# Lornatang/Real_ESRGAN-PyTorch

Hardware: AMD Instinct MI355X
Metric: x4 SR train images/sec (256->1024) (higher is better)
Workload: dtype f16; 1 GPU; RealESRNet x4 L1 train step, RRDBNet 23 blocks, LR 256^2 -> HR 1024^2, batch 16/GPU, degradation=hip, Adam+EMA, GradScaler; global_batch=16, parallelism=dp1

## Files before the change

real_esrgan-pytorch_amd/csrc/build.py:

```python
import os
import subprocess
import sys
from concurrent.futures import ThreadPoolExecutor

HERE = os.path.dirname(os.path.abspath(__file__))
ROOT = os.path.dirname(os.path.dirname(HERE))
SOURCES = ["api.hip", "conv3x3.hip", "conv3x3_ws.hip", "conv3x3_ws_mt1.hip", "conv3x3_ws_mt2.hip", "conv3x3_ws_x2_mt1.hip", "conv3x3_ws_x2_mt2.hip", "conv3x3_ws_sp.hip", "conv3x3_ws_chain.hip", "conv3x3_ws_chain_x2.hip", "wgrad.hip", "pack.hip", "layout.hip", "generator.hip", "degrade.hip", "degrade_int.hip", "disc.hip", "disc_native.hip", "loss.hip", "sustained.hip"]
LIB = os.path.join(HERE, "libresr_hip.so")
HIPCC = os.environ.get("HIPCC", "/opt/rocm/bin/hipcc")
FLAGS = ["--offload-arch=gfx950", "-O3", "-std=c++17", "-fPIC", "-I", os.path.join(ROOT, "include"), "-I", HERE,
         "-Wno-unused-result"]


def _stale(target, deps):
    if not os.path.exists(target):
        return True
    t = os.path.getmtime(target)
    return any(os.path.getmtime(d) > t for d in deps)


def build(force=False, verbose=False):
    hdrs = [os.path.join(HERE, "common.h"), os.path.join(HERE, "conv3x3.h"), os.path.join(HERE, "conv3x3_ws.h"), os.path.join(HERE, "conv3x3_ws_chain.h"), os.path.join(HERE, "wgrad.h"), os.path.join(ROOT, "include", "resr.h"), os.path.join(ROOT, "include", "resr_debug.h"), os.path.abspath(__file__)]
    extra = [s for s in os.listdir(HERE) if s.endswith(".hip") and s not in SOURCES]
    srcs = SOURCES + sorted(extra)
    objs, jobs = [], []
    for s in srcs:
        src = os.path.join(HERE, s)
        obj = os.path.join(HERE, s.replace(".hip", ".o"))
        objs.append(obj)
        if force or _stale(obj, [src] + hdrs):
            cmd = [HIPCC] + FLAGS + ["-c", src, "-o", obj]
            if verbose:
                cmd.insert(1, "-Rpass-analysis=kernel-resource-usage")
            jobs.append(cmd)

    def run(cmd):
        r = subprocess.run(cmd, capture_output=True, text=True)
        return cmd, r

    with ThreadPoolExecutor(max_workers=6) as ex:
        for cmd, r in ex.map(run, jobs):
            if verbose or r.returncode:
                sys.stderr.write(" ".join(cmd) + "\n" + r.stdout + r.stderr)
            if r.returncode:
                raise RuntimeError("hipcc failed: " + " ".join(cmd))
    if force or jobs or _stale(LIB, objs):
        cmd = [HIPCC, "--offload-arch=gfx950", "-shared", "-fPIC", "-o", LIB] + objs
        r = subprocess.run(cmd, capture_output=True, text=True)
        if r.returncode:
            sys.stderr.write(r.stdout + r.stderr)
            raise RuntimeError("link failed")
    return LIB


if __name__ == "__main__":
    print(build(force="--force" in sys.argv, verbose="--verbose" in sys.argv))
```

real_esrgan-pytorch_amd/csrc/generator.hip:

```cpp
#include <stdlib.h>
#include <vector>

#include "common.h"
#include "wgrad.h"

namespace resr {

int conv3x3_dispatch(const ResrConvDesc*, const void*, const void*, const void*, const float*, const void*,
                     const void*, const void*, void*, void*, hipStream_t);
size_t wgrad_batch_partial_bytes(const WgradConv*, int, int, int);
int conv3x3_block_dispatch(int njobs, const ResrConvDesc* d, const void* in0, const void* in1, const void* const* w,
                           const float* const* bias, const void* const* mask, void* const* out, void* const* aux,
                           const ResrConvDesc* d5, const void* w5, const float* bias5, const void* res0_5, const void* res1_5,
                           void* out5, void* chain_state, size_t chain_state_bytes, hipStream_t stream);
size_t conv3x3_chain_state_bytes(int, int, int);
int wgrad_batch(const WgradConv*, int, int, int, int, int, int, int, float*, hipStream_t);
int wgrad_batch_jobs(const WgradConv*, int, int);
int wgrad_batch_quads(const WgradConv*, int, int);
int wgrad_tile_rows(int dtype);
int wgrad_x2_products();
int nchw_to_nhwc_dispatch(const float*, void*, int, int, int, int, int, int, int, const uint8_t*, hipStream_t, long);
int nhwc_to_nchw_dispatch(const void*, float*, int, int, int, int, int, int, int, hipStream_t, long);
int absmax_dispatch(const float*, long, unsigned*, int, hipStream_t);
int nchw_to_nhwc_scaled_dispatch(const float*, void*, int, int, int, int, int, int, int, const uint8_t*, hipStream_t, long, const unsigned*);
int nchw_to_nhwc_q_dispatch(const float*, void*, int, int, int, int, int, int, int, const uint8_t*, hipStream_t, long, const unsigned*, long);
int nhwc_to_nchw_scaled_dispatch(const void*, float*, int, int, int, int, int, int, int, hipStream_t, long, const unsigned*);
int sumpool2x2_dispatch(const void*, void*, const void*, int, int, int, int, int, float, hipStream_t, long, long);
int add_inplace_dispatch(void*, const void*, long, int, hipStream_t, long, long);

namespace {

struct ConvSpec {
    int cout, cin, cin_pad, cout_pad;
    size_t w_off, b_off;
    size_t pk_fwd, pk_bwd;
};

struct Plan {
    ResrGeneratorDesc d;
    int r;
    int h, w;
    int ci_real, ci_pad;
    int nrdb;
    std::vector<ConvSpec> convs;
    size_t n_params;
    size_t pk_fwd_elems, pk_total_elems;
    int i_conv1, i_trunk0, i_conv2, i_up1, i_up2, i_conv3, i_conv4;
    std::vector<size_t> pk_bwd_trunk;
    size_t pk_bwd_conv4, pk_bwd_conv3, pk_bwd_up2, pk_bwd_up1, pk_bwd_conv2, pk_bwd_conv1;
};

int round32(int v) { return (v + 31) / 32 * 32; }

bool plan_mx_bwd(const ResrGeneratorDesc& d) {
    return d.dtype == RESR_F16X2 && d.training && (d.x2_plan & RESR_X2_PLAN_MX_BWD) && !(d.x2_plan & RESR_X2_PLAN_GROWTH_GRAD_STORE_F16);
}
bool plan_mx_wgrad(const ResrGeneratorDesc& d) {
    return plan_mx_bwd(d) && (d.x2_plan & RESR_X2_PLAN_MX_WGRAD) && !(d.x2_plan & RESR_X2_PLAN_F16_BACKWARD);
}
bool plan_mx_tail(const ResrGeneratorDesc& d) { return plan_mx_wgrad(d) && (d.x2_plan & RESR_X2_PLAN_MX_TAIL); }
constexpr int kMxTrainNeeds = RESR_X2_PLAN_GROWTH_F16_INFER | RESR_X2_PLAN_GROWTH_W16_INFER | RESR_X2_PLAN_MX_INFER | RESR_X2_PLAN_F16_BACKWARD;
bool plan_mx_train(const ResrGeneratorDesc& d) {
    return d.dtype == RESR_F16X2 && d.training && (d.x2_plan & RESR_X2_PLAN_MX_TRAIN_FORWARD) && (d.x2_plan & kMxTrainNeeds) == kMxTrainNeeds;
}
bool plan_mx_train_ok(const ResrGeneratorDesc& d) {
    return d.dtype != RESR_F16X2 || !(d.x2_plan & RESR_X2_PLAN_MX_TRAIN_FORWARD) || (d.x2_plan & kMxTrainNeeds) == kMxTrainNeeds;
}
bool plan_mx(const ResrGeneratorDesc& d) {
    const int need = RESR_X2_PLAN_GROWTH_F16_INFER | RESR_X2_PLAN_GROWTH_W16_INFER | RESR_X2_PLAN_MX_INFER;
    return (d.dtype == RESR_F16X2 && !d.training && (d.x2_plan & need) == need) || plan_mx_train(d);
}

bool build_plan(const ResrGeneratorDesc* d, Plan& p) {
    if (!d) return false;
    if (d->upscale != 4 && d->upscale != 2 && d->upscale != 1) return false;
    if (d->n <= 0 || d->h <= 0 || d->w <= 0 || d->n_blocks <= 0 || d->in_channels <= 0 || d->out_channels <= 0) return false;
    p.d = *d;
    p.r = d->upscale == 4 ? 1 : (d->upscale == 2 ? 2 : 4);
    if ((d->h % p.r) || (d->w % p.r)) return false;
    p.h = d->h / p.r;
    p.w = d->w / p.r;
    p.ci_real = d->in_channels * p.r * p.r;
    p.ci_pad = round32(p.ci_real);
    if (p.ci_pad > 64 || d->out_channels > 32) return false;
    p.nrdb = d->n_blocks * 3;
    size_t off = 0;
    auto add = [&](int cout, int cin) {
        ConvSpec c;
        c.cout = cout; c.cin = cin; c.cin_pad = round32(cin); c.cout_pad = round32(cout);
        c.w_off = off; off += (size_t)cout * cin * 9;
        c.b_off = off; off += cout;
        c.pk_fwd = c.pk_bwd = 0;
        p.convs.push_back(c);
        return (int)p.convs.size() - 1;
    };
    p.i_conv1 = add(64, p.ci_real);
    p.i_trunk0 = (int)p.convs.size();
    for (int r = 0; r < p.nrdb; ++r)
        for (int k = 1; k <= 5; ++k) add(k < 5 ? 32 : 64, 64 + 32 * (k - 1));
    p.i_conv2 = add(64, 64);
    p.i_up1 = add(64, 64);
    p.i_up2 = add(64, 64);
    p.i_conv3 = add(64, 64);
    p.i_conv4 = add(d->out_channels, 64);
    p.n_params = off;
    size_t pk = 0;
    for (auto& c : p.convs) {
        c.pk_fwd = pk;
        pk += (size_t)(c.cin_pad / 32) * 9 * (c.cout_pad / 32) * 1024;
    }
    p.pk_fwd_elems = pk;
    auto bwd_simple = [&](int idx) {
        const ConvSpec& c = p.convs[idx];
        const size_t o = pk;
        pk += (size_t)(c.cout_pad / 32) * 9 * (c.cin_pad / 32) * 1024;
        return o;
    };
    p.pk_bwd_conv4 = bwd_simple(p.i_conv4);
    p.pk_bwd_conv3 = bwd_simple(p.i_conv3);
    p.pk_bwd_up2 = bwd_simple(p.i_up2);
    p.pk_bwd_up1 = bwd_simple(p.i_up1);
    p.pk_bwd_conv2 = bwd_simple(p.i_conv2);
    p.pk_bwd_conv1 = bwd_simple(p.i_conv1);
    p.pk_bwd_trunk.resize((size_t)p.nrdb * 5);
    for (int r = 0; r < p.nrdb; ++r)
        for (int ps = 0; ps < 5; ++ps) {
            p.pk_bwd_trunk[(size_t)r * 5 + ps] = pk;
            pk += (size_t)(2 + ps) * 9 * (ps < 4 ? 1 : 2) * 1024;
        }
    p.pk_total_elems = pk;
    return true;
}

struct Bufs {
    char* chain;
    size_t chain_bytes;
    char* x_in;
    std::vector<char*> ws;
    char *bits_u2, *bits_c3;
    std::vector<char*> bits;
    char* out1;
    int out1_stride;
    char *trunk_out, *feat, *u1, *u2, *c3;
    uint8_t* ymask;
    char *g4, *gA, *gB, *gM1, *gF, *gT[4], *gS[3], *gxin;
    float* partial;
    size_t partial_bytes;
    unsigned* gscale;
    size_t total;
};

int splits_for(const Plan& p, int npairs, int h, int w, int nquads = 0) {
    if (p.d.wgrad_splits > 0) return p.d.wgrad_splits;
    const int th = wgrad_tile_rows(p.d.dtype);
    const long tiles = (long)((w + 31) / 32) * ((h + th - 1) / th) * p.d.n;
    if (p.d.dtype == RESR_F16X2 && nquads > 0 && tiles >= 64 && !getenv("RESR_X2_WGRAD_OLD_SPLITS")) {
        long best_s = 8;
        double best = 1e30;
        for (long s = 8; s <= 256 && s <= tiles / 2; s += 8) {
            const long rounds = (nquads * (s / 8) + 31) / 32;
            const double cost = rounds * ((double)tiles / s * 2.9 + 8.0) + (double)npairs * s * 0.0185;
            if (cost < best) { best = cost; best_s = s; }
        }
        return (int)best_s;
    }
    long s;
    if (p.d.dtype != RESR_F32) {
        s = 512 / ((npairs + 3) / 4);
        if (s >= 16) s &= ~7L;
        if (s > 256) s = 256;
    } else {
        s = 768 / npairs;
        if (s > 128) s = 128;
    }
    if (s > tiles / 2) s = tiles / 2;
    if (s < 1) s = 1;
    return (int)s;
}

void carve(const Plan& p, char* base, Bufs& b) {
    const size_t es = elem_size(p.d.dtype) * (act_tensors(p.d.dtype) + (plan_mx(p.d) ? 1 : 0));
// ... 294 lines not shown
                outs4[k - 1] = cur + (size_t)(2 + (k - 1)) * plane * es; signs4[k - 1] = signs;
            }
            const ConvSpec& c = p.convs[p.i_trunk0 + r * 5 + 4];
            const bool last = r == p.nrdb - 1;
            char* dst = last ? b.trunk_out : b.ws[(r + 1) % nws];
            ResrConvDesc cd = conv_desc(p, N, h, w, 192, 192, 32, 0, 64, 64, 32, 0);
            cd.in0_chunk_stride = plane;
            cd.out_chunk_stride = plane;
            cd.in0_lo_offset = lo_ws; cd.out_lo_offset = last ? lo_t : lo_ws;
            if (growth_single) { cd.x2_pair_chunks = 2; if (growth_w16) cd.flags |= RESR_CONV_SINGLE_W16; }
            MXP(cd, c, 2 * lo_ws, last ? 2 * lo_t : 2 * lo_ws);
            if (mxw && !last) cd.out_q_offset = 2 * lo_ws;
            cd.s0 = 0.2f; cd.t0 = 1.f; cd.res0_stride = 32; cd.res0_chunk_stride = plane; cd.res0_lo_offset = lo_ws;
            const char* res1 = nullptr;
            if (r % 3 == 2) {
                res1 = b.ws[(r - 2) % nws];
                cd.s1 = 0.2f; cd.t1 = 1.f; cd.res1_stride = 32; cd.res1_chunk_stride = plane; cd.res1_lo_offset = lo_ws;
            }
            RUN(conv3x3_block_dispatch(4, cds, cur, nullptr, ws4, bs4, nullptr, outs4, signs4, &cd, W(c), Bias(c), cur, res1, dst, b.chain, b.chain_bytes, st));
        }
    }
    {
        const ConvSpec& c = p.convs[p.i_conv2];
        ResrConvDesc cd = conv_desc(p, N, h, w, 64, 64, 32, 0, 64, 64, 64, 0);
        cd.in0_chunk_stride = plane;
        cd.res0_stride = b.out1_stride;
        cd.res0_chunk_stride = b.out1 == b.ws[0] ? plane : 0;
        cd.out_stride = 32; cd.out_chunk_stride = plane;
        cd.in0_lo_offset = lo_t; cd.res0_lo_offset = lo_out1; cd.out_lo_offset = lo_t;
        MXP(cd, c, 2 * lo_t, 2 * lo_t);
        RUN(conv3x3_dispatch(&cd, b.trunk_out, nullptr, W(c), Bias(c), b.out1, nullptr, nullptr, b.feat, nullptr, st));
    }
    {
        const ConvSpec& c = p.convs[p.i_up1];
        ResrConvDesc cd = conv_desc(p, N, 2 * h, 2 * w, 64, 64, 32, 0, 64, 64, 32, RESR_CONV_LRELU | RESR_CONV_UPSAMPLE_IN);
        cd.in0_chunk_stride = plane; cd.out_chunk_stride = 4 * plane;
        cd.in0_lo_offset = lo_t; cd.out_lo_offset = LO(2, 4L * plane);
        MXP(cd, c, 2 * lo_t, 2 * LO(2, 4L * plane));
        if (mxt) cd.out_q_offset = 2 * LO(2, 4L * plane);
        RUN(conv3x3_dispatch(&cd, b.feat, nullptr, W(c), Bias(c), nullptr, nullptr, nullptr, b.u1, nullptr, st));
    }
    {
        const ConvSpec& c = p.convs[p.i_up2];
        ResrConvDesc cd = conv_desc(p, N, 4 * h, 4 * w, 64, 64, 32, 0, 64, 64, 32, RESR_CONV_LRELU | RESR_CONV_UPSAMPLE_IN);
        cd.in0_chunk_stride = 4 * plane; cd.out_chunk_stride = 16 * plane;
        cd.in0_lo_offset = LO(2, 4L * plane); cd.out_lo_offset = LO(2, 16L * plane);
        if (d->training) cd.flags |= RESR_CONV_WRITE_SIGNBITS;
        MXP(cd, c, 2 * LO(2, 4L * plane), 2 * LO(2, 16L * plane));
        if (mxt) cd.out_q_offset = 2 * LO(2, 16L * plane);
        RUN(conv3x3_dispatch(&cd, b.u1, nullptr, W(c), Bias(c), nullptr, nullptr, nullptr, b.u2, b.bits_u2, st));
    }
    {
        const ConvSpec& c = p.convs[p.i_conv3];
        ResrConvDesc cd = conv_desc(p, N, 4 * h, 4 * w, 64, 64, 32, 0, 64, 64, 32, RESR_CONV_LRELU);
        cd.in0_chunk_stride = 16 * plane; cd.out_chunk_stride = 16 * plane;
        cd.in0_lo_offset = LO(2, 16L * plane); cd.out_lo_offset = LO(2, 16L * plane);
        if (d->training) cd.flags |= RESR_CONV_WRITE_SIGNBITS;
        MXP(cd, c, 2 * LO(2, 16L * plane), 0);
        if (mxt) cd.out_q_offset = 2 * LO(2, 16L * plane);
        RUN(conv3x3_dispatch(&cd, b.u2, nullptr, W(c), Bias(c), nullptr, nullptr, nullptr, b.c3, b.bits_c3, st));
    }
    {
        const ConvSpec& c = p.convs[p.i_conv4];
        ResrConvDesc cd = conv_desc(p, N, 4 * h, 4 * w, 64, 64, 32, 0, c.cout, c.cout_pad, 0,
                                    RESR_CONV_CLAMP01 | RESR_CONV_OUT_NCHW_F32);
        cd.in0_chunk_stride = 16 * plane;
        cd.in0_lo_offset = LO(2, 16L * plane);
        RUN(conv3x3_dispatch(&cd, b.c3, nullptr, W(c), Bias(c), nullptr, nullptr, nullptr, y, b.ymask, st));
    }
    return RESR_OK;
}

int generator_backward(const ResrGeneratorDesc* d, const float* gy, const float* params, const void* packed,
                       void* workspace, size_t workspace_bytes, float* grad, float* gx, hipStream_t st,
                       void* const* events, int n_events) {
    (void)params;
    Plan p;
    if (!build_plan(d, p)) return fail(RESR_ERR_ARG, "generator_backward: bad descriptor");
    if (!plan_mx_train_ok(*d)) return fail(RESR_ERR_ARG, "generator_backward: x2_plan MX_TRAIN_FORWARD (2048) needs bits 1 + 32 + 64 + 256");
    if (n_events != 0 && (!events || n_events != d->n_blocks + 2))
        return fail(RESR_ERR_ARG, "generator_backward: grad_ready_events needs n_blocks + 2 = %d events, got %d", d->n_blocks + 2, n_events);
    auto ready = [&](int i) -> int {
        if (n_events == 0) return RESR_OK;
        if (!events[i]) return fail(RESR_ERR_ARG, "generator_backward: null event %d", i);
        if (hipEventRecord((hipEvent_t)events[i], st) != hipSuccess) return fail(RESR_ERR_LAUNCH, "generator_backward: hipEventRecord");
        return RESR_OK;
    };
    if (!d->training) return fail(RESR_ERR_ARG, "generator_backward: forward was not run with training=1");
    if (!gy || !packed || !workspace || !grad) return fail(RESR_ERR_ARG, "generator_backward: null argument");
    Bufs b;
    carve(p, (char*)workspace, b);
    if (b.total > workspace_bytes) return fail(RESR_ERR_WORKSPACE, "generator_backward: workspace %zu < %zu", workspace_bytes, b.total);
    const bool f16bwd = d->dtype == RESR_F16X2 && (d->x2_plan & RESR_X2_PLAN_F16_BACKWARD);
    const int dt = f16bwd ? (int)RESR_F16 : d->dtype;
    Plan pb = p;
    pb.d.dtype = dt;
    const size_t es = elem_size(dt);
    const bool x2 = dt == RESR_F16X2;
    const size_t wes = es * (x2 ? 3 : 1);
    const int wm = x2 ? wgrad_x2_products() : 1;
    const char* no_prescale = getenv("RESR_X2_NO_GRAD_PRESCALE");
    const char* pre_t = getenv("RESR_X2_GRAD_PRESCALE_LOG2");
    const int pre_log2 = pre_t ? atoi(pre_t) : 6;
    const unsigned* gsc = (dt != RESR_F32 && !no_prescale) ? b.gscale : nullptr;
    const bool mxb = plan_mx_bwd(*d) && !f16bwd;
    const bool mxw = plan_mx_wgrad(*d) && mxb;
    const bool mxt = plan_mx_tail(*d) && mxw;
    const bool gg_single = x2 && (d->x2_plan & RESR_X2_PLAN_GROWTH_GRAD_F16);
    const bool gg_store_single = gg_single && (d->x2_plan & RESR_X2_PLAN_GROWTH_GRAD_STORE_F16);
    const int wx_pairs = (x2 && (d->x2_plan & RESR_X2_PLAN_GROWTH_ACT_F16_WGRAD)) ? 2 : 0;
    const char* pk = (const char*)packed;
    const int N = d->n, h = p.h, w = p.w;
    const int H4 = 4 * h, W4 = 4 * w, H2 = 2 * h, W2 = 2 * w;
    if ((long)N * h * w * 32 * 16 > 0x7fffffffL) return fail(RESR_ERR_ARG, "generator: batch x resolution too large for 32-bit chunk strides");
    const int plane = N * h * w * 32;
    const int pl2 = 4 * plane, pl4 = 16 * plane;
    auto LO = [&](long planes, long pl) -> long { return x2 ? planes * pl : 0; };
    const long lo_ws = LO(6, plane), lo_t = LO(2, plane), lo_gs = LO(4, plane), lo_2 = LO(2, pl2), lo_4 = LO(2, pl4), lo_g4 = LO(1, pl4);
    const long lo_xin = x2 ? (long)N * h * w * p.ci_pad : 0;

    auto wconv = [&](const ConvSpec& c, const void* x0, int cin, int s0, const void* g, int gstride, float scale,
                     long x_lo, long g_lo) {
        WgradConv wc;
        wc.x0 = x0; wc.cin = cin; wc.in0_stride = s0; wc.cin_real = c.cin;
        wc.g = g; wc.cout = c.cout; wc.cout_pad = c.cout_pad; wc.g_stride = gstride;
        wc.x_chunk_stride = wc.g_chunk_stride = 0;
        wc.x_lo_off = x_lo; wc.g_lo_off = g_lo; wc.x_s2d_c = 0; wc.g_lo_bias_only = 0;
        wc.dw = grad + c.w_off; wc.db = grad + c.b_off; wc.scale = scale;
        wc.unscale = gsc;
        return wc;
    };
    auto wgrad_run = [&](const WgradConv* wc, int nconv, int hh, int ww, int flags) -> int {
        const int njobs = wgrad_batch_jobs(wc, nconv, dt);
        const int splits = splits_for(pb, njobs, hh, ww, x2 ? wgrad_batch_quads(wc, nconv, dt) : 0);
        if (wgrad_batch_partial_bytes(wc, nconv, splits, dt) > b.partial_bytes)
            return fail(RESR_ERR_WORKSPACE, "wgrad slab buffer too small");
        return wgrad_batch(wc, nconv, N, hh, ww, dt, flags, splits, b.partial, st);
    };
    auto wgrad = [&](const ConvSpec& c, int hh, int ww, const void* x0, int cin, int s0, const void* g, int gstride,
                     int flags, float scale, long x_chunk, long g_chunk, long x_lo, long g_lo, long x_q = 0, long g_q = 0) -> int {
        WgradConv wc = wconv(c, x0, cin, s0, g, gstride, scale, x_lo, g_lo);
        wc.x_chunk_stride = x_chunk; wc.g_chunk_stride = g_chunk;
        wc.x_q_off = x_q; wc.g_q_off = g_q;
        return wgrad_run(&wc, 1, hh, ww, flags);
    };
    auto dgrad = [&](int hh, int ww, int cin0, int s0, int cin, int s1, int cout, int cout_pad, int out_stride, int flags,
                     long lo0, long lo1, long lo_out) {
        ResrConvDesc cd = conv_desc(pb, N, hh, ww, cin, cin0, s0, s1, cout, cout_pad, out_stride, flags | RESR_CONV_NO_BIAS);
        cd.in0_lo_offset = lo0; cd.in1_lo_offset = lo1; cd.out_lo_offset = lo_out;
        return cd;
    };

    if (gsc) RUN(absmax_dispatch(gy, (long)N * d->out_channels * H4 * W4, b.gscale, pre_log2, st));
    RUN(nchw_to_nhwc_q_dispatch(gy, b.g4, N, d->out_channels, H4, W4, 1, 32, dt, b.ymask, st, lo_g4, gsc, mxt ? 2 * lo_g4 : 0L));
    const char* pk_mx = mxb ? pk + generator_mx_offset(d) : nullptr;
    auto MXT = [&](ResrConvDesc& cd, size_t pk_off, long in_q, long out_q) {
        if (!mxt) return;
        cd.flags |= RESR_CONV_MX_PAIRS;
        cd.in0_q_offset = in_q; cd.out_q_offset = out_q;
        cd.w_mx_offset = (int64_t)((pk_mx + pk_off * 2) - (pk + pk_off * wes));
    };
    {
        const ConvSpec& c = p.convs[p.i_conv4];
        RUN(wgrad(c, H4, W4, b.c3, 64, 32, b.g4, 32, 0, 1.f, pl4, 0, lo_4, lo_g4, mxt ? 2 * lo_4 : 0, mxt ? 2 * lo_g4 : 0));
        ResrConvDesc cd = dgrad(H4, W4, 32, 32, 32, 0, 64, 64, 32, RESR_CONV_MASK | RESR_CONV_MASK_BITS, lo_g4, 0, lo_4);
        cd.out_chunk_stride = pl4;
        MXT(cd, p.pk_bwd_conv4, 2 * lo_g4, 2 * lo_4);
        RUN(conv3x3_dispatch(&cd, b.g4, nullptr, pk + p.pk_bwd_conv4 * wes, nullptr, nullptr, nullptr, b.bits_c3, b.gA, nullptr, st));
    }
    {
        const ConvSpec& c = p.convs[p.i_conv3];
        RUN(wgrad(c, H4, W4, b.u2, 64, 32, b.gA, 32, 0, 1.f, pl4, pl4, lo_4, lo_4, mxt ? 2 * lo_4 : 0, mxt ? 2 * lo_4 : 0));
        ResrConvDesc cd = dgrad(H4, W4, 64, 32, 64, 0, 64, 64, 32, RESR_CONV_MASK | RESR_CONV_MASK_BITS, lo_4, 0, lo_4);
        cd.in0_chunk_stride = pl4; cd.out_chunk_stride = pl4;
        MXT(cd, p.pk_bwd_conv3, 2 * lo_4, 2 * lo_4);
        RUN(conv3x3_dispatch(&cd, b.gA, nullptr, pk + p.pk_bwd_conv3 * wes, nullptr, nullptr, nullptr, b.bits_u2, b.gB, nullptr, st));
    }
    if (debug_stop() == 1) return RESR_OK;
    {
        const ConvSpec& c = p.convs[p.i_up2];
        RUN(wgrad(c, H4, W4, b.u1, 64, 32, b.gB, 32, RESR_CONV_UPSAMPLE_IN, 1.f, pl2, pl4, lo_2, lo_4, mxt ? 2 * lo_2 : 0, mxt ? 2 * lo_4 : 0));
        ResrConvDesc cd = dgrad(H4, W4, 64, 32, 64, 0, 64, 64, 32, 0, lo_4, 0, lo_4);
        cd.in0_chunk_stride = pl4; cd.out_chunk_stride = pl4;
        MXT(cd, p.pk_bwd_up2, 2 * lo_4, 0);
        RUN(conv3x3_dispatch(&cd, b.gB, nullptr, pk + p.pk_bwd_up2 * wes, nullptr, nullptr, nullptr, nullptr, b.gA, nullptr, st));
        for (int q = 0; q < 2; ++q)
            RUN(sumpool2x2_dispatch(b.gA + (size_t)q * pl4 * es, b.gM1 + (size_t)q * pl2 * es, b.u1 + (size_t)q * pl2 * es,
                                    N, H2, W2, 32, dt, 0.2f, st, lo_4, lo_2));
    }
    if (debug_stop() == 2) return RESR_OK;
    {
        const ConvSpec& c = p.convs[p.i_up1];
        RUN(wgrad(c, H2, W2, b.feat, 64, 32, b.gM1, 32, RESR_CONV_UPSAMPLE_IN, 1.f, plane, pl2, lo_t, lo_2));
        ResrConvDesc cd = dgrad(H2, W2, 64, 32, 64, 0, 64, 64, 32, 0, lo_2, 0, lo_2);
        cd.in0_chunk_stride = pl2; cd.out_chunk_stride = pl2;
        RUN(conv3x3_dispatch(&cd, b.gM1, nullptr, pk + p.pk_bwd_up1 * wes, nullptr, nullptr, nullptr, nullptr, b.gA, nullptr, st));
        for (int q = 0; q < 2; ++q)
            RUN(sumpool2x2_dispatch(b.gA + (size_t)q * pl2 * es, b.gF + (size_t)q * plane * es, nullptr, N, h, w, 32, dt, 0.2f, st,
                                    lo_2, lo_t));
    }
    if (debug_stop() == 3) return RESR_OK;
    int cur = 0;
    {
        const ConvSpec& c = p.convs[p.i_conv2];
        RUN(wgrad(c, h, w, b.trunk_out, 64, 32, b.gF, 32, 0, 1.f, plane, plane, lo_t, lo_t));
        ResrConvDesc cd = dgrad(h, w, 64, 32, 64, 0, 64, 64, 32, 0, lo_t, 0, lo_t);
        cd.in0_chunk_stride = plane; cd.out_chunk_stride = plane;
        if (mxb) cd.out_q_offset = 2 * lo_t;
        RUN(conv3x3_dispatch(&cd, b.gF, nullptr, pk + p.pk_bwd_conv2 * wes, nullptr, nullptr, nullptr, nullptr, b.gT[0], nullptr, st));
    }
    auto MXB = [&](ResrConvDesc& cd, size_t pk_off, long out_q) {
        if (!mxb) return;
        cd.flags |= RESR_CONV_MX_PAIRS;
        cd.x2_pair_chunks = 0;
        cd.in0_q_offset = 2 * lo_t; cd.in1_q_offset = 2 * lo_gs; cd.out_q_offset = out_q;
        cd.w_mx_offset = (int64_t)((pk_mx + pk_off * 2) - (pk + pk_off * wes));
    };
    RUN(ready(0));
    int e_idx = 0;
    const bool batch_rrdb = 78 * wm <= kWgradMaxJobs && !getenv("RESR_WGRAD_PER_BLOCK");
    WgradConv wc[15];
    for (int r = p.nrdb - 1; r >= 0; --r) {
        const int pos = r % 3;
        if (pos == 2) e_idx = cur;
        const char* gin = b.gT[cur];
        const char* act = b.ws[r];
        char* gS = b.gS[pos];
        const float fold = pos == 2 ? 0.04f : 0.2f;
        WgradConv* wcb = wc + (batch_rrdb ? 5 * pos : 0);
        wcb[4] = wconv(p.convs[p.i_trunk0 + r * 5 + 4], act, 192, 32, gin, 32, fold, lo_ws, lo_t);
        wcb[4].x_chunk_stride = plane; wcb[4].g_chunk_stride = plane;
        wcb[4].x_pair_chunks = wx_pairs;
        wcb[4].x_single_g_hi = (wx_pairs && (d->x2_plan & RESR_X2_PLAN_GROWTH_ACT_G_HI_WGRAD)) ? 1 : 0;
        if (mxw) { wcb[4].x_q_off = 2 * lo_ws; wcb[4].g_q_off = 2 * lo_t; }
        ResrConvDesc cds[4];
        const void* ws4[4];
        const void* masks4[4];
        void* outs4[4];
        for (int ps = 0; ps < 4; ++ps) {
            const int k = 4 - ps;
            const int cin = 64 + 32 * ps;
            ResrConvDesc cd = dgrad(h, w, 64, 32, cin, 32, 32, 32, 32, RESR_CONV_MASK | RESR_CONV_MASK_BITS, lo_t, lo_gs, lo_gs);
            cd.in0_chunk_stride = plane; cd.in1_chunk_stride = plane;
            if (gg_single) cd.x2_pair_chunks = 2;
            if (gg_store_single) cd.flags |= RESR_CONV_OUT_SINGLE;
            MXB(cd, p.pk_bwd_trunk[(size_t)r * 5 + ps], 2 * lo_gs);
            char* out = gS + (size_t)ps * plane * es;
            const char* mask = b.bits[r] + (size_t)(k - 1) * N * h * w * sizeof(uint32_t);
            cds[ps] = cd; ws4[ps] = pk + p.pk_bwd_trunk[(size_t)r * 5 + ps] * wes; masks4[ps] = mask; outs4[ps] = out;
            const ConvSpec& c = p.convs[p.i_trunk0 + r * 5 + k - 1];
            wcb[k - 1] = wconv(c, act, c.cin, 32, out, 32, 1.f, lo_ws, gg_store_single ? 0 : lo_gs);
            wcb[k - 1].x_chunk_stride = plane;
            wcb[k - 1].g_lo_bias_only = (gg_single && !gg_store_single) ? 1 : 0;
            wcb[k - 1].x_pair_chunks = wx_pairs;
            if (mxw) { wcb[k - 1].x_q_off = 2 * lo_ws; wcb[k - 1].g_q_off = 2 * lo_gs; }
        }
        {
            int nxt = (cur + 1) & 3;
            if (nxt == e_idx && pos != 2) nxt = (nxt + 1) & 3;
            ResrConvDesc cd = dgrad(h, w, 64, 32, 192, 32, 64, 64, 32, 0, lo_t, lo_gs, lo_t);
            cd.in0_chunk_stride = plane; cd.in1_chunk_stride = plane; cd.out_chunk_stride = plane;
            if (gg_single) cd.x2_pair_chunks = 2;
            const char* res0 = gin;
            const char* res1 = nullptr;
            cd.res0_stride = 32; cd.res0_chunk_stride = plane; cd.s0 = 1.f; cd.res0_lo_offset = lo_t;
            cd.t0 = pos == 2 ? 0.2f : 1.f;
            if (pos == 0) { res1 = b.gT[e_idx]; cd.res1_stride = 32; cd.res1_chunk_stride = plane; cd.s1 = 1.f; cd.t1 = 1.f; cd.res1_lo_offset = lo_t; }
            MXB(cd, p.pk_bwd_trunk[(size_t)r * 5 + 4], 2 * lo_t);
            RUN(conv3x3_block_dispatch(4, cds, gin, gS, ws4, nullptr, masks4, outs4, nullptr, &cd,
                                       pk + p.pk_bwd_trunk[(size_t)r * 5 + 4] * wes, nullptr, res0, res1, b.gT[nxt], b.chain, b.chain_bytes, st));
            cur = nxt;
        }
        if (!batch_rrdb) RUN(wgrad_run(wc, 5, h, w, 0));
        else if (pos == 0) RUN(wgrad_run(wc, 15, h, w, 0));
        if (pos == 0) RUN(ready(1 + (d->n_blocks - 1 - r / 3)));
    }
    if (debug_stop() == 4) return RESR_OK;
    RUN(add_inplace_dispatch(b.gT[cur], b.gF, (long)N * h * w * 64, dt, st, lo_t, lo_t));
    {
        const ConvSpec& c = p.convs[p.i_conv1];
        RUN(wgrad(c, h, w, b.x_in, p.ci_pad, p.ci_pad, b.gT[cur], 32, 0, 1.f, 0, plane, lo_xin, lo_t));
        RUN(ready(d->n_blocks + 1));
        if (gx) {
            ResrConvDesc cd = dgrad(h, w, 64, 32, 64, 0, p.ci_pad, p.ci_pad, p.ci_pad, 0, lo_t, 0, lo_xin);
            cd.in0_chunk_stride = plane;
            RUN(conv3x3_dispatch(&cd, b.gT[cur], nullptr, pk + p.pk_bwd_conv1 * wes, nullptr, nullptr, nullptr, nullptr, b.gxin, nullptr, st));
            RUN(nhwc_to_nchw_scaled_dispatch(b.gxin, gx, N, d->in_channels, d->h, d->w, p.r, p.ci_pad, dt, st, lo_xin, gsc));
        }
    }
    return RESR_OK;
}

}
```

Before: 131.0 images/sec.

## Add compact 4-channel tail backward kernels for final 3-output conv

Result: no change. 132.1 images/sec (median of 6 runs) (+0.8%).

```diff
diff --git a/real_esrgan-pytorch_amd/csrc/build.py b/real_esrgan-pytorch_amd/csrc/build.py
--- a/real_esrgan-pytorch_amd/csrc/build.py
+++ b/real_esrgan-pytorch_amd/csrc/build.py
@@ -5,7 +5,7 @@
 
 HERE = os.path.dirname(os.path.abspath(__file__))
 ROOT = os.path.dirname(os.path.dirname(HERE))
-SOURCES = ["api.hip", "conv3x3.hip", "conv3x3_ws.hip", "conv3x3_ws_mt1.hip", "conv3x3_ws_mt2.hip", "conv3x3_ws_x2_mt1.hip", "conv3x3_ws_x2_mt2.hip", "conv3x3_ws_sp.hip", "conv3x3_ws_chain.hip", "conv3x3_ws_chain_x2.hip", "wgrad.hip", "pack.hip", "layout.hip", "generator.hip", "degrade.hip", "degrade_int.hip", "disc.hip", "disc_native.hip", "loss.hip", "sustained.hip"]
+SOURCES = ["api.hip", "conv3x3.hip", "conv3x3_ws.hip", "conv3x3_ws_mt1.hip", "conv3x3_ws_mt2.hip", "conv3x3_ws_x2_mt1.hip", "conv3x3_ws_x2_mt2.hip", "conv3x3_ws_sp.hip", "conv3x3_ws_chain.hip", "conv3x3_ws_chain_x2.hip", "wgrad.hip", "tail_bwd.hip", "pack.hip", "layout.hip", "generator.hip", "degrade.hip", "degrade_int.hip", "disc.hip", "disc_native.hip", "loss.hip", "sustained.hip"]
 LIB = os.path.join(HERE, "libresr_hip.so")
 HIPCC = os.environ.get("HIPCC", "/opt/rocm/bin/hipcc")
 FLAGS = ["--offload-arch=gfx950", "-O3", "-std=c++17", "-fPIC", "-I", os.path.join(ROOT, "include"), "-I", HERE,
diff --git a/real_esrgan-pytorch_amd/csrc/generator.hip b/real_esrgan-pytorch_amd/csrc/generator.hip
--- a/real_esrgan-pytorch_amd/csrc/generator.hip
+++ b/real_esrgan-pytorch_amd/csrc/generator.hip
@@ -27,6 +27,9 @@
 int nhwc_to_nchw_scaled_dispatch(const void*, float*, int, int, int, int, int, int, int, hipStream_t, long, const unsigned*);
 int sumpool2x2_dispatch(const void*, void*, const void*, int, int, int, int, int, float, hipStream_t, long, long);
 int add_inplace_dispatch(void*, const void*, long, int, hipStream_t, long, long);
+int nchw_to_nhwc4_dispatch(const float*, void*, int, int, int, int, const uint8_t*, const unsigned*, hipStream_t);
+int conv4_dgrad_dispatch(const void*, const void*, const void*, void*, int, int, int, long, float, hipStream_t);
+int conv4_wgrad_dispatch(const void*, long, const void*, int, int, int, int, float*, float*, float, const unsigned*, float*, size_t, hipStream_t);
 
 namespace {
 
@@ -627,7 +630,11 @@
     };
 
     if (gsc) RUN(absmax_dispatch(gy, (long)N * d->out_channels * H4 * W4, b.gscale, pre_log2, st));
-    RUN(nchw_to_nhwc_q_dispatch(gy, b.g4, N, d->out_channels, H4, W4, 1, 32, dt, b.ymask, st, lo_g4, gsc, mxt ? 2 * lo_g4 : 0L));
+    const char* tail_legacy = getenv("RESR_TAIL_LEGACY");
+    const bool compact4 = dt == RESR_F16 && !mxt && d->out_channels == 3 &&
+                          !(tail_legacy && (tail_legacy[0] == '1' || tail_legacy[0] == 'a' || tail_legacy[0] == 'A'));
+    if (compact4) RUN(nchw_to_nhwc4_dispatch(gy, b.g4, N, d->out_channels, H4, W4, b.ymask, gsc, st));
+    else RUN(nchw_to_nhwc_q_dispatch(gy, b.g4, N, d->out_channels, H4, W4, 1, 32, dt, b.ymask, st, lo_g4, gsc, mxt ? 2 * lo_g4 : 0L));
     const char* pk_mx = mxb ? pk + generator_mx_offset(d) : nullptr;
     auto MXT = [&](ResrConvDesc& cd, size_t pk_off, long in_q, long out_q) {
         if (!mxt) return;
@@ -635,7 +642,11 @@
         cd.in0_q_offset = in_q; cd.out_q_offset = out_q;
         cd.w_mx_offset = (int64_t)((pk_mx + pk_off * 2) - (pk + pk_off * wes));
     };
-    {
+    if (compact4) {
+        const ConvSpec& c = p.convs[p.i_conv4];
+        RUN(conv4_wgrad_dispatch(b.c3, pl4, b.g4, N, H4, W4, c.cin, grad + c.w_off, grad + c.b_off, 1.f, gsc, b.partial, b.partial_bytes, st));
+        RUN(conv4_dgrad_dispatch(b.g4, pk + p.pk_bwd_conv4 * wes, b.bits_c3, b.gA, N, H4, W4, pl4, 0.2f, st));
+    } else {
         const ConvSpec& c = p.convs[p.i_conv4];
         RUN(wgrad(c, H4, W4, b.c3, 64, 32, b.g4, 32, 0, 1.f, pl4, 0, lo_4, lo_g4, mxt ? 2 * lo_4 : 0, mxt ? 2 * lo_g4 : 0));
         ResrConvDesc cd = dgrad(H4, W4, 32, 32, 32, 0, 64, 64, 32, RESR_CONV_MASK | RESR_CONV_MASK_BITS, lo_g4, 0, lo_4);
diff --git a/real_esrgan-pytorch_amd/csrc/tail_bwd.hip b/real_esrgan-pytorch_amd/csrc/tail_bwd.hip
--- /dev/null
+++ b/real_esrgan-pytorch_amd/csrc/tail_bwd.hip
@@ -0,0 +1,355 @@
+#include "common.h"
+
+namespace resr {
+
+namespace {
+
+typedef _Float16 h2 __attribute__((ext_vector_type(2)));
+
+constexpr int kTaps = 27;
+constexpr int kTailSlab = 27 * 64 + 4;
+
+__global__ __launch_bounds__(256) void nchw_to_nhwc4_kernel(const float* __restrict__ src, half_t* __restrict__ dst, int n, int c,
+                                                            int h, int w, const uint8_t* __restrict__ mask,
+                                                            const unsigned* __restrict__ amax, int vec) {
+    const int x = (int)(blockIdx.x * 256u + threadIdx.x) * 4;
+    if (x >= w) return;
+    const float pre = amax ? grad_prescale(*amax, false) : 1.f;
+    for (int b = (int)blockIdx.z; b < n; b += (int)gridDim.z)
+    for (int y = (int)blockIdx.y; y < h; y += (int)gridDim.y) {
+        half_t o[4][4];
+#pragma unroll
+        for (int ch = 0; ch < 4; ++ch) {
+            float v[4] = {0.f, 0.f, 0.f, 0.f};
+            if (ch < c) {
+                const size_t q = (((size_t)b * c + ch) * h + y) * w + x;
+                if (vec) {
+                    const float4v s = *reinterpret_cast<const float4v*>(src + q);
+                    const unsigned mk = mask ? *reinterpret_cast<const unsigned*>(mask + q) : 0x01010101u;
+#pragma unroll
+                    for (int e = 0; e < 4; ++e) {
+                        v[e] = s[e] * pre;
+                        if (mask) v[e] = ((mk >> (8 * e)) & 0xffu) ? v[e] : 0.f;
+                    }
+                } else {
+#pragma unroll
+                    for (int e = 0; e < 4; ++e) {
+                        if (x + e >= w) continue;
+                        v[e] = src[q + e] * pre;
+                        if (mask) v[e] = mask[q + e] ? v[e] : 0.f;
+                    }
+                }
+            }
+#pragma unroll
+            for (int e = 0; e < 4; ++e) o[e][ch] = (half_t)v[e];
+        }
+        half_t* d = dst + (((size_t)b * h + y) * w + x) * 4;
+        if (vec) {
+            *reinterpret_cast<uint4*>(d) = *reinterpret_cast<const uint4*>(&o[0][0]);
+            *reinterpret_cast<uint4*>(d + 8) = *reinterpret_cast<const uint4*>(&o[2][0]);
+        } else {
+#pragma unroll
+            for (int e = 0; e < 4; ++e)
+                if (x + e < w) *reinterpret_cast<uint2*>(d + e * 4) = *reinterpret_cast<const uint2*>(&o[e][0]);
+        }
+    }
+}
+
+constexpr int kDgRows = 4;
+
+__global__ __launch_bounds__(256) void conv4_dgrad_kernel(const half_t* __restrict__ g4c, const half_t* __restrict__ wpk,
+                                                          const unsigned* __restrict__ bits, half_t* __restrict__ out, int h, int w,
+                                                          long chunk_stride, float slope) {
+    __shared__ unsigned wl[64][16];
+    for (int idx = threadIdx.x; idx < 64 * 16; idx += 256) {
+        const int ci = idx >> 4, pr = idx & 15;
+        h2 v = {(half_t)0.f, (half_t)0.f};
+#pragma unroll
+        for (int s = 0; s < 2; ++s) {
+            const int i = 2 * pr + s;
+            if (i < kTaps) {
+                const int tap = i / 3, co = i - tap * 3;
+                v[s] = wpk[co + 8 * (ci & 31) + 512 * (ci >> 5) + 2048 * tap];
+            }
+        }
+        wl[ci][pr] = __builtin_bit_cast(unsigned, v);
+    }
+    __syncthreads();
+    const int lane = threadIdx.x & 63, wave = threadIdx.x >> 6;
+    const int x = (int)blockIdx.x * 64 + lane;
+    const int y0 = (int)blockIdx.y * 16 + wave * kDgRows;
+    const int n = (int)blockIdx.z;
+    if (x >= w || y0 >= h) return;
+    uint2 nb[kDgRows + 2][3];
+#pragma unroll
+    for (int r = 0; r < kDgRows + 2; ++r)
+#pragma unroll
+        for (int c = 0; c < 3; ++c) {
+            const int yy = y0 + r - 1, xx = x + c - 1;
+            const bool ok = yy >= 0 && yy < h && xx >= 0 && xx < w;
+            const size_t p = ((size_t)n * h + (ok ? yy : 0)) * w + (ok ? xx : 0);
+            const uint2 v = *reinterpret_cast<const uint2*>(g4c + p * 4);
+            nb[r][c] = ok ? v : make_uint2(0u, 0u);
+        }
+    h2 vp[kDgRows][14];
+#pragma unroll
+    for (int t = 0; t < kDgRows; ++t) {
+        half_t e[28];
+#pragma unroll
+        for (int ty = 0; ty < 3; ++ty)
+#pragma unroll
+            for (int tx = 0; tx < 3; ++tx) {
+                const half4 q = __builtin_bit_cast(half4, nb[t + ty][tx]);
+                e[(ty * 3 + tx) * 3 + 0] = q[0];
+                e[(ty * 3 + tx) * 3 + 1] = q[1];
+                e[(ty * 3 + tx) * 3 + 2] = q[2];
+            }
+        e[27] = (half_t)0.f;
+#pragma unroll
+        for (int k = 0; k < 14; ++k) vp[t][k] = h2{e[2 * k], e[2 * k + 1]};
+    }
+    unsigned mw[kDgRows][2];
+#pragma unroll
+    for (int t = 0; t < kDgRows; ++t) {
+        const int yy = y0 + t < h ? y0 + t : h - 1;
+        const size_t p = ((size_t)n * h + yy) * w + x;
+        mw[t][0] = bits[p * 2];
+        mw[t][1] = bits[p * 2 + 1];
+    }
+#pragma unroll 1
+    for (int grp = 0; grp < 8; ++grp) {
+        float acc[kDgRows][8];
+#pragma unroll
+        for (int c = 0; c < 8; ++c) {
+            const int ci = grp * 8 + c;
+            uint4 wq[4];
+#pragma unroll
+            for (int k = 0; k < 4; ++k) wq[k] = *reinterpret_cast<const uint4*>(&wl[ci][4 * k]);
+            const unsigned* wv = reinterpret_cast<const unsigned*>(wq);
+#pragma unroll
+            for (int t = 0; t < kDgRows; ++t) {
+                float s = 0.f;
+#pragma unroll
+                for (int k = 0; k < 14; ++k) s = __builtin_amdgcn_fdot2(vp[t][k], __builtin_bit_cast(h2, wv[k]), s, false);
+                acc[t][c] = s;
+            }
+        }
+        const int m = grp >> 2, cb = (grp & 3) * 8;
+#pragma unroll
+        for (int t = 0; t < kDgRows; ++t) {
+            if (y0 + t >= h) continue;
+            const unsigned byte = mw[t][m] >> cb;
+            half8 o;
+#pragma unroll
+            for (int c = 0; c < 8; ++c) o[c] = (half_t)(acc[t][c] * (((byte >> c) & 1u) ? 1.f : slope));
+            const size_t p = ((size_t)n * h + y0 + t) * w + x;
+            *reinterpret_cast<half8*>(out + (size_t)m * chunk_stride + p * 32 + cb) = o;
+        }
+    }
+}
+
+struct TailWgradArgs {
+    const half_t* x;
+    const half_t* g;
+    float* partial;
+    long x_chunk;
+    int n, h, w, tiles_x, ntiles;
+};
+
+__global__ __launch_bounds__(256) void conv4_wgrad_kernel(const TailWgradArgs a) {
+    __shared__ __attribute__((aligned(16))) char smem[16384];
+    half_t* xs = reinterpret_cast<half_t*>(smem);
+    half_t* gs = reinterpret_cast<half_t*>(smem + 8192);
+    const int tid = threadIdx.x, lane = tid & 63, wave = tid >> 6;
+    const int nwg = (int)gridDim.x;
+
+    uint4 rx[2];
+    uint2 rg;
+    auto fetch = [&](int tile) {
+        const int tx = tile % a.tiles_x, row = tile / a.tiles_x;
+        const int y = row % a.h, x0 = tx * 64;
+#pragma unroll
+        for (int i = 0; i < 2; ++i) {
+            const int px = tid >> 2, c16 = tid & 3;
+            const bool ok = x0 + px < a.w;
+            const size_t p = (size_t)row * a.w + (ok ? x0 + px : 0);
+            const uint4 v = *reinterpret_cast<const uint4*>(a.x + (size_t)i * a.x_chunk + p * 32 + c16 * 8);
+            rx[i] = ok ? v : make_uint4(0u, 0u, 0u, 0u);
+        }
+        {
+            const int t = tid < 198 ? tid : 0;
+            const int r = t / 66, j = t - r * 66;
+            const int yy = y + r - 1, xx = x0 + j - 1;
+            const bool ok = tid < 198 && yy >= 0 && yy < a.h && xx >= 0 && xx < a.w;
+            const size_t p = ok ? (size_t)(row + r - 1) * a.w + xx : 0;
+            const uint2 v = *reinterpret_cast<const uint2*>(a.g + p * 4);
+            rg = ok ? v : make_uint2(0u, 0u);
+        }
+    };
+    double bsum[3] = {0.0, 0.0, 0.0};
+    auto commit = [&]() {
+#pragma unroll
+        for (int i = 0; i < 2; ++i) *reinterpret_cast<uint4*>(xs + i * 2048 + (tid >> 2) * 32 + (tid & 3) * 8) = rx[i];
+        if (tid < 198) {
+            *reinterpret_cast<uint2*>(gs + tid * 4) = rg;
+            if (tid >= 67 && tid < 131) {
+                const half4 q = __builtin_bit_cast(half4, rg);
+                bsum[0] += (double)q[0]; bsum[1] += (double)q[1]; bsum[2] += (double)q[2];
+            }
+        }
+    };
+
+    float16v acc[2];
+#pragma unroll
+    for (int m = 0; m < 2; ++m)
+#pragma unroll
+        for (int r = 0; r < 16; ++r) acc[m][r] = 0.f;
+
+    const int i = lane & 31, kg = lane >> 5;
+    const int tap = i / 3, co = i - tap * 3, ky = tap / 3, kx = tap - ky * 3;
+    const bool arow = i < kTaps;
+    const half_t* ga = gs + (((arow ? 2 - ky : 0) * 66) + wave * 16 + kg * 8 + 2 - (arow ? kx : 0)) * 4 + (arow ? co : 0);
+    const half_t* xb = xs + (wave * 16 + kg * 8) * 32 + i;
+
+    int tile = (int)blockIdx.x;
+    if (tile < a.ntiles) fetch(tile);
+    for (; tile < a.ntiles; tile += nwg) {
+        __syncthreads();
+        commit();
+        __syncthreads();
+        if (tile + nwg < a.ntiles) fetch(tile + nwg);
+        half8 fa, fb0, fb1;
+#pragma unroll
+        for (int e = 0; e < 8; ++e) {
+            fa[e] = arow ? ga[e * 4] : (half_t)0.f;
+            fb0[e] = xb[e * 32];
+            fb1[e] = xb[2048 + e * 32];
+        }
+        acc[0] = __builtin_amdgcn_mfma_f32_32x32x16_f16(fa, fb0, acc[0], 0, 0, 0);
+        acc[1] = __builtin_amdgcn_mfma_f32_32x32x16_f16(fa, fb1, acc[1], 0, 0, 0);
+    }
+
+    float* red = reinterpret_cast<float*>(smem);
+    double* redb = reinterpret_cast<double*>(smem);
+    float* slab = a.partial + (size_t)blockIdx.x * kTailSlab;
+#pragma unroll
+    for (int m = 0; m < 2; ++m) {
+        __syncthreads();
+#pragma unroll
+        for (int r = 0; r < 16; ++r) red[(wave * 16 + r) * 64 + lane] = acc[m][r];
+        __syncthreads();
+#pragma unroll
+        for (int k = 0; k < 4; ++k) {
+            const int e = tid + k * 256;
+            const int r = e >> 6, l = e & 63;
+            const float s = (red[e] + red[1024 + e]) + (red[2048 + e] + red[3072 + e]);
+            const int row = (r & 3) + 8 * (r >> 2) + 4 * (l >> 5), ci = m * 32 + (l & 31);
+            if (row < kTaps) slab[row * 64 + ci] = s;
+        }
+    }
+    __syncthreads();
+    if (tid >= 67 && tid < 131) {
+#pragma unroll
+        for (int c = 0; c < 3; ++c) redb[c * 64 + tid - 67] = bsum[c];
+    }
+    __syncthreads();
+    if (tid < 3) {
+        double s = 0.0;
+        for (int k = 0; k < 64; ++k) s += redb[tid * 64 + k];
+        slab[kTaps * 64 + tid] = (float)s;
+    }
+}
+
+__global__ __launch_bounds__(256) void conv4_wgrad_reduce_kernel(const float* __restrict__ partial, int nslabs, float* __restrict__ dw,
+                                                                 float* __restrict__ db, int cin, float scale,
+                                                                 const unsigned* __restrict__ unscale) {
+    __shared__ double red[8][32];
+    const int lane = threadIdx.x & 31, g = threadIdx.x >> 5;
+    const int e = (int)blockIdx.x * 32 + lane;
+    constexpr int kOut = kTaps * 64 + 3;
+    double sd = 0.0;
+    if (e < kOut) {
+        constexpr int U = 8;
+        const float* p = partial + e;
+        for (int k0 = g; k0 < nslabs; k0 += 8 * U) {
+            float v[U];
+#pragma unroll
+            for (int u = 0; u < U; ++u) {
+                const int k = k0 + 8 * u;
+                v[u] = k < nslabs ? p[(size_t)k * kTailSlab] : 0.f;
+            }
+#pragma unroll
+            for (int u = 0; u < U; ++u)
+                if (k0 + 8 * u < nslabs) sd += (double)v[u];
+        }
+    }
+    red[g][lane] = sd;
+    __syncthreads();
+    if (g != 0 || e >= kOut) return;
+    float s = (float)(((red[0][lane] + red[1][lane]) + (red[2][lane] + red[3][lane])) + ((red[4][lane] + red[5][lane]) + (red[6][lane] + red[7][lane]))) * scale;
+    if (unscale) {
+        const unsigned mb = *unscale;
+        s *= grad_prescale(mb, true);
+        if (grad_prescale_lifted(mb) && !(__builtin_fabsf(s) <= 3.0e38f)) const_cast<unsigned*>(unscale)[2] = 1u;
+    }
+    if (e < kTaps * 64) {
+        const int row = e >> 6, ci = e & 63, tap = row / 3, co = row - tap * 3;
+        if (ci < cin) dw[((size_t)co * cin + ci) * 9 + tap] = s;
+    } else if (db) {
+        db[e - kTaps * 64] = s;
+    }
+}
+
+}
+
+int nchw_to_nhwc4_dispatch(const float* src, void* dst, int n, int c, int h, int w, const uint8_t* mask, const unsigned* amax,
+                           hipStream_t stream) {
+    if (!src || !dst || n <= 0 || c <= 0 || c > 4 || h <= 0 || w <= 0) return fail(RESR_ERR_ARG, "nchw_to_nhwc4: bad argument");
+    const int vec = (w % 4 == 0 && !((size_t)src & 15) && !((size_t)dst & 15) && !((size_t)mask & 3)) ? 1 : 0;
+    const dim3 grid((unsigned)(((w + 3) / 4 + 255) / 256), (unsigned)(h > 65535 ? 65535 : h), (unsigned)(n > 65535 ? 65535 : n));
+    hipLaunchKernelGGL(nchw_to_nhwc4_kernel, grid, dim3(256), 0, stream, src, (half_t*)dst, n, c, h, w, mask, amax, vec);
+    RESR_CHECK_LAUNCH("nchw_to_nhwc4_kernel");
+    return RESR_OK;
+}
+
+size_t conv4_wgrad_slab_bytes() { return (size_t)kTailSlab * sizeof(float); }
+
+int conv4_dgrad_dispatch(const void* g4c, const void* wpk, const void* bits, void* out, int n, int h, int w, long out_chunk,
+                         float slope, hipStream_t stream) {
+    if (!g4c || !wpk || !bits || !out || n <= 0 || h <= 0 || w <= 0 || n > 65535 || (h + 15) / 16 > 65535)
+        return fail(RESR_ERR_ARG, "conv4_dgrad: bad argument");
+    const dim3 grid((unsigned)((w + 63) / 64), (unsigned)((h + 15) / 16), (unsigned)n);
+    prof_before(stream);
+    hipLaunchKernelGGL(conv4_dgrad_kernel, grid, dim3(256), 0, stream, (const half_t*)g4c, (const half_t*)wpk, (const unsigned*)bits,
+                       (half_t*)out, h, w, out_chunk, slope);
+    RESR_CHECK_LAUNCH("conv4_dgrad_kernel");
+    const double px = (double)n * h * w;
+    prof_after(stream, 23340, 2.0 * 27 * 64 * px, px * (8.0 + 8.0 + 128.0));
+    return RESR_OK;
+}
+
+int conv4_wgrad_dispatch(const void* x, long x_chunk, const void* g4c, int n, int h, int w, int cin, float* dw, float* db, float scale,
+                         const unsigned* unscale, float* partial, size_t partial_bytes, hipStream_t stream) {
+    if (!x || !g4c || !dw || !partial || n <= 0 || h <= 0 || w <= 0 || cin != 64) return fail(RESR_ERR_ARG, "conv4_wgrad: bad argument");
+    const long tiles_x = (w + 63) / 64;
+    const long ntiles = tiles_x * h * n;
+    if (ntiles > 0x7fffffffL) return fail(RESR_ERR_ARG, "conv4_wgrad: too many tiles");
+    long nwg = (long)(partial_bytes / conv4_wgrad_slab_bytes());
+    if (nwg > 2048) nwg = 2048;
+    if (nwg > ntiles) nwg = ntiles;
+    if (nwg < 1) return fail(RESR_ERR_WORKSPACE, "conv4_wgrad: slab buffer too small");
+    TailWgradArgs a;
+    a.x = (const half_t*)x; a.g = (const half_t*)g4c; a.partial = partial; a.x_chunk = x_chunk;
+    a.n = n; a.h = h; a.w = w; a.tiles_x = (int)tiles_x; a.ntiles = (int)ntiles;
+    prof_before(stream);
+    hipLaunchKernelGGL(conv4_wgrad_kernel, dim3((unsigned)nwg), dim3(256), 0, stream, a);
+    RESR_CHECK_LAUNCH("conv4_wgrad_kernel");
+    const double px = (double)n * h * w;
+    prof_after(stream, 50043, 2.0 * 27 * 64 * px, px * (128.0 + 24.0));
+    hipLaunchKernelGGL(conv4_wgrad_reduce_kernel, dim3((kTaps * 64 + 3 + 31) / 32), dim3(256), 0, stream, partial, (int)nwg, dw, db, cin,
+                       scale, unscale);
+    RESR_CHECK_LAUNCH("conv4_wgrad_reduce_kernel");
+    return RESR_OK;
+}
+
+}
```
